# wtsi-svi/ReadServer

Hardware: AMD Instinct MI355X
Metric: 31-mer backward-search queries/sec on popBWT, counted as (query x shard) backward searches/s (higher is better)
Workload: dtype u64

## Files before the change

readserver_amd/csrc/search_lines.hip:

```cpp
#include <hip/hip_runtime.h>
#include <stdint.h>
#include <stdlib.h>
#include <string.h>

#include <type_traits>

#include "kernels.h"
#include "line_format.h"
#include "rank_device.h"
#include "wave_lines.h"

namespace rsb {


__device__ __forceinline__ ulonglong2 start_record(const shard_view &ix, const uint64_t *pq, uint32_t k) {
    ulonglong2 rec;
    const uint64_t last = pq[(k - 1u) >> 5];
    if (view_uses_ktab(ix, k)) {
        const uint32_t T = ix.ktab_depth;
        const uint32_t off = 2u * (k - T);
        const uint32_t w0 = off >> 6, sh = off & 63u;
        uint64_t bits = (w0 == ((k - 1u) >> 5) ? last : pq[w0]) >> sh;
        if (sh + 2u * T > 64u) bits |= last << (64u - sh);
        const uint64_t e = ktab_entry(ix.ktab, ix.ktab_fmt, T, ix.ktab_stride, bits & ((1ull << (2u * T)) - 1ull));
        const uint32_t width = (uint32_t)(e >> COUNT_BITS);
        if (width != KTAB_WIDE && (e & COUNT_MASK) + width <= ix.n) {
            rec.x = e & COUNT_MASK;
            rec.y = rec.x + width - 1ull;
            return rec;
        }
    }
    const uint32_t b = (uint32_t)((last >> (2u * ((k - 1u) & 31u))) & 3u) + 1u;
    rec.x = ix.C[b] | INIT_FALLBACK;
    rec.y = ix.C[b] + ix.total[b] - 1ull;
    return rec;
}

__global__ void __launch_bounds__(256)
search_init_kernel(const shard_view *__restrict__ shards, uint32_t nshards, const uint64_t *__restrict__ packed,
                   const uint8_t *__restrict__ valid, size_t Q, uint32_t k, uint32_t wpq,
                   ulonglong2 *__restrict__ init) {
    const size_t i = (size_t)blockIdx.x * blockDim.x + threadIdx.x;
    if (i >= Q * nshards) return;
    const size_t q = i / nshards, s = i - q * nshards;
    ulonglong2 rec;
    if (valid[q] == 0) {
        rec.x = INIT_INVALID;
        rec.y = 0;
    } else {
        rec = start_record(shards[s], packed + q * wpq, k);
    }
    init[s * Q + q] = rec;
}

__global__ void __launch_bounds__(256)
search_init_var_kernel(const shard_view *__restrict__ shards, uint32_t nshards, const uint64_t *__restrict__ packed,
                       const uint8_t *__restrict__ valid, const uint32_t *__restrict__ len, size_t Q, uint32_t wpq,
                       ulonglong2 *__restrict__ init) {
    const size_t i = (size_t)blockIdx.x * blockDim.x + threadIdx.x;
    if (i >= Q * nshards) return;
    const size_t q = i / nshards, s = i - q * nshards;
    const uint32_t L = len[q];
    ulonglong2 rec;
    if (valid[q] == 0 || L == 0u) {
        rec.x = INIT_INVALID;
        rec.y = 0;
    } else {
        const shard_view &ix = shards[s];
        const uint64_t *pq = packed + q * wpq;
        bool tabulated = false;
        if (view_uses_ktab(ix, L)) {
            const uint32_t T = ix.ktab_depth;
            const uint32_t off = 2u * (L - T);
            const uint32_t w0 = off >> 6, sh = off & 63u;
            uint64_t bits = pq[w0] >> sh;
            if (sh + 2u * T > 64u) bits |= pq[w0 + 1u] << (64u - sh);
            const uint64_t e = ktab_entry(ix.ktab, ix.ktab_fmt, T, ix.ktab_stride, bits & ((1ull << (2u * T)) - 1ull));
            const uint32_t width = (uint32_t)(e >> COUNT_BITS);
            if (width != KTAB_WIDE && (e & COUNT_MASK) + width <= ix.n) {
                rec.x = (e & COUNT_MASK) | ((uint64_t)(L - T) << COUNT_BITS) | INIT_EXPLICIT | INIT_VAR;
                rec.y = (e & COUNT_MASK) + width - 1ull;
                tabulated = true;
            }
        }
        if (!tabulated) {
            const uint32_t b = (uint32_t)((pq[(L - 1u) >> 5] >> (2u * ((L - 1u) & 31u))) & 3u) + 1u;
            rec.x = ix.C[b] | ((uint64_t)(L - 1u) << COUNT_BITS) | INIT_EXPLICIT | INIT_VAR | INIT_NOCHECK;
            rec.y = ix.C[b] + ix.total[b] - 1ull;
        }
    }
    init[s * Q + q] = rec;
}

__global__ void __launch_bounds__(256)
search_init_tiled_kernel(const shard_view *__restrict__ shards, uint32_t nshards, const uint64_t *__restrict__ packed,
                         const uint8_t *__restrict__ valid, size_t Q, uint32_t k, uint32_t wpq, uint32_t V,
                         ulonglong2 *__restrict__ init) {
    __shared__ ulonglong2 tile[256];
    const size_t q0 = (size_t)blockIdx.x * V;
    const uint32_t t = threadIdx.x;
    {
        const uint32_t v = t / nshards, s = t - v * nshards;
        if (v < V && q0 + v < Q) {
            const size_t q = q0 + v;
            ulonglong2 rec;
            if (valid[q] == 0) {
                rec.x = INIT_INVALID;
                rec.y = 0;
            } else {
                rec = start_record(shards[s], packed + q * wpq, k);
            }
            tile[v * nshards + s] = rec;
        }
    }
    __syncthreads();
    {
        const uint32_t s = t / V, v = t - s * V;
        if (s < nshards && q0 + v < Q) init[(size_t)s * Q + q0 + v] = tile[v * nshards + s];
    }
}

constexpr uint32_t INIT_U = 4;
__global__ void __launch_bounds__(256)
search_init_tiled4_kernel(const shard_view *__restrict__ shards, uint32_t nshards, const uint64_t *__restrict__ packed,
                          const uint8_t *__restrict__ valid, size_t Q, uint32_t k, uint32_t V, ulonglong2 *__restrict__ init) {
    __shared__ ulonglong2 tile[INIT_U][256];
    const size_t q0 = (size_t)blockIdx.x * V * INIT_U;
    const uint32_t t = threadIdx.x;
    {
        const uint32_t v = t / nshards, s = t - v * nshards;
        if (v < V) {
            const shard_view &ix = shards[s];
            const bool tab = view_uses_ktab(ix, k);
            const uint32_t T = ix.ktab_depth, off = tab ? 2u * (k - T) : 0u;
            const uint64_t *ktab = ix.ktab;
            const uint32_t fmt = ix.ktab_fmt, stride = ix.ktab_stride;
            const uint64_t n = ix.n;
            uint8_t ok[INIT_U];
            uint64_t word[INIT_U], e[INIT_U];
#pragma unroll
            for (uint32_t u = 0; u < INIT_U; ++u) {
                const size_t q = q0 + (size_t)u * V + v;
                const bool in = q < Q;
                ok[u] = in ? valid[q] : (uint8_t)2;
                word[u] = in ? packed[q] : 0ull;
            }
#pragma unroll
            for (uint32_t u = 0; u < INIT_U; ++u)
                e[u] = (tab && ok[u] == 1) ? ktab_entry(ktab, fmt, T, stride, (word[u] >> off) & ((1ull << (2u * T)) - 1ull)) : ~0ull;
#pragma unroll
            for (uint32_t u = 0; u < INIT_U; ++u) {
                if (ok[u] == 2) continue;
                ulonglong2 rec;
                const uint32_t width = (uint32_t)(e[u] >> COUNT_BITS);
                if (ok[u] == 0) {
                    rec.x = INIT_INVALID;
                    rec.y = 0;
                } else if (tab && width != KTAB_WIDE && (e[u] & COUNT_MASK) + width <= n) {
                    rec.x = e[u] & COUNT_MASK;
                    rec.y = rec.x + width - 1ull;
                } else {
                    const uint32_t b = (uint32_t)((word[u] >> (2u * ((k - 1u) & 31u))) & 3u) + 1u;
                    rec.x = ix.C[b] | INIT_FALLBACK;
                    rec.y = ix.C[b] + ix.total[b] - 1ull;
                }
                tile[u][v * nshards + s] = rec;
            }
        }
    }
    __syncthreads();
    {
        const uint32_t s = t / V, v = t - s * V;
        if (s < nshards) {
#pragma unroll
            for (uint32_t u = 0; u < INIT_U; ++u) {
                const size_t q = q0 + (size_t)u * V + v;
                if (q < Q) init[(size_t)s * Q + q] = tile[u][v * nshards + s];
            }
        }
    }
}

__global__ void __launch_bounds__(256)
search_init_1mm_kernel(const shard_view *__restrict__ shards, uint32_t nshards, const uint64_t *__restrict__ vpacked,
                       const uint8_t *__restrict__ vvalid, size_t mv, uint32_t k, uint32_t wpq, uint32_t V,
                       const ulonglong2 *__restrict__ trace, uint32_t trace_n,
                       ulonglong2 *__restrict__ init) {
    const size_t t_ = (size_t)blockIdx.x * blockDim.x + threadIdx.x;
    if (t_ >= mv * nshards) return;
    const size_t i = t_ / nshards, s = t_ - i * nshards;
    ulonglong2 rec;
    if (vvalid[i] == 0) {
        rec.x = INIT_INVALID;
        rec.y = 0;
    } else {
        const size_t q = i / V;
        const uint32_t v = (uint32_t)(i - q * V);
        const uint32_t pos = v ? (v - 1u) / 3u : ~0u;
        if (pos < trace_n) {
            const ulonglong2 t = trace[(s * (mv / V) + q) * trace_n + pos];
            rec.x = (t.x & COUNT_MASK) | ((uint64_t)pos << COUNT_BITS) | INIT_EXPLICIT;
            rec.y = t.y;
        } else {
            rec = start_record(shards[s], vpacked + i * wpq, k);
        }
    }
    init[s * mv + i] = rec;
}

enum { WORK_STEPS = 0, WORK_OCC = 1, WORK_LINES = 2, WORK_KTAB = 3, WORK_PHASE0 = 4, WORK_PASSES = 10, WORK_HOPS = 11, WORK_SOLO = 12 };
enum { WORK_UNSTAGED = 15 };

template <bool COUNT_WORK, bool COUNTS_ONLY, bool LONGK, int ROLE>
__global__ void __launch_bounds__(64 * WG_WAVES, RSB_MIN_WGS_PER_CU)
search_lines_kernel(const shard_view *__restrict__ shards, uint32_t nshards, const uint64_t *__restrict__ packed,
                    const ulonglong2 *__restrict__ init, unsigned long long *__restrict__ next_query,
                    size_t Q, uint32_t k, uint32_t wpq,
                    uint64_t *__restrict__ out_lower, uint64_t *__restrict__ out_upper,
                    unsigned long long *__restrict__ work,
                    ulonglong2 *__restrict__ trace, uint32_t trace_n, uint32_t qchunk, uint32_t pairs) {
    __shared__ uint4 s_stage[WG_WAVES][64 * SLOT_U4];
    const uint32_t lane = threadIdx.x & 63u;
    const uint32_t wave = threadIdx.x >> 6;
    const uint32_t side = lane >> 5;
    uint4 *stage = s_stage[wave];
    const uint32_t stage_lds = __builtin_amdgcn_readfirstlane((uint32_t)(uintptr_t)(lds_void_ptr)stage);
    const uint32_t swz = lane & 7u;
    const lds_u32 *own_row = reinterpret_cast<const lds_u32 *>(stage + (lane & 7u) * 64u + (lane >> 3) * SLOT_U4);
#define MINE(d) (mine0 + (((((uint32_t)(d)) >> 2) ^ swz) << 2) + (((uint32_t)(d)) & 3u))

    unsigned long long w_steps = 0, w_occ = 0, w_lines = 0, w_hops = 0, w_ktab = 0;
    unsigned long long ph[6] = {0, 0, 0, 0, 0, 0}, stamp = 0, passes = 0;
#define STAMP(i)                                                        \
    if (COUNT_WORK) {                                                   \
        __builtin_amdgcn_sched_barrier(0);                              \
        const unsigned long long now_ = __builtin_amdgcn_s_memtime();   \
        asm volatile("s_waitcnt lgkmcnt(0)" ::: "memory");              \
        ph[i] += now_ - stamp;                                          \
        stamp = now_;                                                   \
        __builtin_amdgcn_sched_barrier(0);                              \
    }
    if (COUNT_WORK) stamp = __builtin_amdgcn_s_memtime();

    uint32_t sid = blockIdx.x % nshards;
    for (uint32_t visited = 0; visited < nshards; ++visited, sid = (sid + 1u == nshards) ? 0u : sid + 1u) {
        const shard_view *sv = shards + sid;
        const char *lines_bytes = reinterpret_cast<const char *>(sv->lines);
        const uint32_t S = sv->sp.S;
        const double inv = sv->sp.inv;
        const uint32_t nlines = (uint32_t)sv->nlines;
        const bool ktab = view_uses_ktab(*sv, k);
        const int j_table = ktab ? (int)(k - sv->ktab_depth) - 1 : (int)k - 2;
        const uint32_t w_table = j_table > 0 ? (uint32_t)j_table >> 5 : 0u;
        const ulonglong2 *init_s = init + (size_t)sid * Q;
        uint64_t *out_lo = out_lower + (size_t)sid * Q * (pairs ? 2u : 1u);
        uint64_t *out_up = (COUNTS_ONLY || pairs) ? nullptr : out_upper + (size_t)sid * Q;
        unsigned long long *pool = next_query + (size_t)sid * POOL_STRIDE;
        if (visited != 0u && __hip_atomic_load(pool, __ATOMIC_RELAXED, __HIP_MEMORY_SCOPE_AGENT) >= (unsigned long long)Q) continue;
        ulonglong2 *trace_s = trace ? trace + (size_t)sid * Q * trace_n : nullptr;
        unsigned long long *hit_map = pairs == 2u ? reinterpret_cast<unsigned long long *>(out_upper) + (size_t)sid * hit_map_words(Q) : nullptr;
        uint32_t ctab_lo, ctab_hi;
        {
            const uint64_t c1 = sv->C[1], c2 = sv->C[2], c3 = sv->C[3], c4 = sv->C[4];
// ... 252 lines not shown
                has_n = true;
            }
            if (alive && done) {
                if (trace && side == 0u) {
                    for (int jj = j < (int)trace_n ? j : (int)trace_n - 1; jj >= 0; --jj)
                        trace_s[q * trace_n + (uint32_t)jj] = make_ulonglong2(lo, hi);
                }
                if (side == 0u) {
                    if (COUNTS_ONLY) {
                        if (hi >= lo) out_lo[q] = hi - lo + 1ull;
                    } else if (pairs == 2u) {
                        if (lo <= hi) {
                            reinterpret_cast<ulonglong2 *>(out_lo)[q] = make_ulonglong2(lo, hi);
                            atomicOr(hit_map + (q >> 6), 1ull << (q & 63u));
                        }
                    } else if (pairs) {
#ifdef RSB_NT_RESULTS
                        __builtin_nontemporal_store(lo, &out_lo[2 * q]);
                        __builtin_nontemporal_store(hi, &out_lo[2 * q + 1]);
#else
                        reinterpret_cast<ulonglong2 *>(out_lo)[q] = make_ulonglong2(lo, hi);
#endif
                    } else {
                        out_lo[q] = lo;
                        out_up[q] = hi;
                    }
                }
                has_q = false;
            }
            STAMP(5)
            if (COUNT_WORK) ++passes;
        }
    }
    if (COUNT_WORK) {
        if (lane == 0u) {
            for (int i = 0; i < 6; ++i) atomicAdd(&work[WORK_PHASE0 + i], ph[i]);
            atomicAdd(&work[WORK_PASSES], passes);
        }
        if (w_steps) atomicAdd(&work[WORK_STEPS], w_steps);
        if (w_occ) atomicAdd(&work[WORK_OCC], w_occ);
        if (w_lines) atomicAdd(&work[WORK_LINES], w_lines);
        if (w_ktab) atomicAdd(&work[WORK_KTAB], w_ktab);
        if (w_hops) atomicAdd(&work[WORK_HOPS], w_hops);
    }
#undef MINE
#undef STAMP
}

}
#include "search_solo.h"
namespace rsb {

static int search_kernel_choice() {
    static const int choice = [] {
        const char *e = getenv("RSBWT_SEARCH_KERNEL");
        if (e && !strcmp(e, "pair")) return SEARCH_PAIR;
        if (e && !strcmp(e, "solo")) return SEARCH_SOLO;
        return SEARCH_AUTO;
    }();
    return choice;
}

static size_t wave_wgs_per_cu() {
    static const size_t v = (size_t)knob_int("RSBWT_WAVE_WGS_PER_CU", 1, INT_MAX, RSB_MIN_WGS_PER_CU);
    return v;
}

static size_t search_cap(int num_cus, size_t wgs_per_cu) {
    static const size_t spare = (size_t)knob_int("RSBWT_SEARCH_SPARE_WGS", 1, LLONG_MAX, 0);
    return resident_cap(num_cus, wgs_per_cu, spare);
}

template <class F>
static void with_flag(bool b, F &&f) {
    if (b) f(std::true_type{});
    else f(std::false_type{});
}
#define FLAG(x) decltype(x)::value

template <bool CW, bool CO>
static void launch_solo(int grid, hipStream_t stream, const shard_view *shards, uint32_t nshards, const uint64_t *pk,
                        const ulonglong2 *init, const uint8_t *valid, unsigned long long *ctr, size_t Q, uint32_t k, uint32_t wpq,
                        uint64_t *lo, uint64_t *up, unsigned long long *work, ulonglong2 *trace, uint32_t trace_n,
                        uint32_t pairs, bool fused) {
    const uint32_t qchunk = plan_draw(1024, 64, (size_t)grid * WG_WAVES, 4, Q * nshards);
    static const bool no_staged = knob_set("RSBWT_NO_STAGED_RESULTS");
    const bool staged = !CO && pairs != 2u && !no_staged;
    static const bool count_unstaged = knob_set("RSBWT_COUNT_UNSTAGED");
    const uint32_t pa = pairs | (staged ? SOLO_STAGED_RESULTS : 0u) | (CW && count_unstaged ? SOLO_COUNT_UNSTAGED : 0u);
    const size_t dyn = staged ? SOLO_RESULTS_LDS : 0u;
    if (fused)
        hipLaunchKernelGGL((search_solo_kernel<CW, CO, false, true>), dim3(grid), dim3(64 * WG_WAVES), dyn, stream, shards, nshards,
                           pk, init, valid, ctr, Q, k, wpq, lo, up, work, trace, trace_n, qchunk, pa);
    else if (wpq > 1)
        hipLaunchKernelGGL((search_solo_kernel<CW, CO, true>), dim3(grid), dim3(64 * WG_WAVES), dyn, stream, shards, nshards,
                           pk, init, valid, ctr, Q, k, wpq, lo, up, work, trace, trace_n, qchunk, pa);
    else
        hipLaunchKernelGGL((search_solo_kernel<CW, CO, false>), dim3(grid), dim3(64 * WG_WAVES), dyn, stream, shards, nshards,
                           pk, init, valid, ctr, Q, k, wpq, lo, up, work, trace, trace_n, qchunk, pa);
}

template <bool CW, bool CO>
static void launch_k(int grid, hipStream_t stream, const shard_view *shards, uint32_t nshards, const uint64_t *pk,
                     const ulonglong2 *init, unsigned long long *ctr, size_t Q, uint32_t k, uint32_t wpq,
                     uint64_t *lo, uint64_t *up, unsigned long long *work, ulonglong2 *trace, uint32_t trace_n,
                     uint32_t pairs) {
    const uint32_t qchunk = plan_draw(1024, 32, (size_t)grid * WG_WAVES, 4, Q * nshards);
    if (wpq > 1)
        hipLaunchKernelGGL((search_lines_kernel<CW, CO, true, 0>), dim3(grid), dim3(64 * WG_WAVES), 0, stream, shards, nshards,
                           pk, init, ctr, Q, k, wpq, lo, up, work, trace, trace_n, qchunk, pairs);
    else
        hipLaunchKernelGGL((search_lines_kernel<CW, CO, false, 0>), dim3(grid), dim3(64 * WG_WAVES), 0, stream, shards, nshards,
                           pk, init, ctr, Q, k, wpq, lo, up, work, trace, trace_n, qchunk, pairs);
}

static void launch_init(const shard_view *d_shards, uint32_t nshards, const uint64_t *pk, const uint8_t *vd, size_t Q, uint32_t k,
                        uint32_t wpq, ulonglong2 *init, hipStream_t stream) {
    static const bool untiled = knob_set("RSBWT_INIT_UNTILED");
    static const bool one_per_thread = knob_set("RSBWT_INIT_ONE_PER_THREAD");
    if (nshards >= 2u && nshards <= 256u && !untiled && wpq == 1u && !one_per_thread) {
        const uint32_t V = 256u / nshards;
        hipLaunchKernelGGL(search_init_tiled4_kernel, dim3((unsigned)((Q + (size_t)V * INIT_U - 1) / ((size_t)V * INIT_U))), dim3(256), 0, stream,
                           d_shards, nshards, pk, vd, Q, k, V, init);
    } else if (nshards >= 2u && nshards <= 256u && !untiled) {
        const uint32_t V = 256u / nshards;
        hipLaunchKernelGGL(search_init_tiled_kernel, dim3((unsigned)((Q + V - 1) / V)), dim3(256), 0, stream, d_shards, nshards, pk, vd, Q,
                           k, wpq, V, init);
    } else {
        const size_t nrec = Q * nshards;
        hipLaunchKernelGGL(search_init_kernel, dim3((unsigned)((nrec + 255) / 256)), dim3(256), 0, stream, d_shards, nshards, pk, vd, Q, k,
                           wpq, init);
    }
}

hipError_t launch_search_init_var(const shard_view *d_shards, uint32_t nshards, const void *d_packed, const void *d_valid,
                                  const void *d_len, size_t Q, uint32_t wpq, void *d_init, hipStream_t stream) {
    if (Q == 0 || nshards == 0) return hipSuccess;
    const size_t nrec = Q * nshards;
    hipLaunchKernelGGL(search_init_var_kernel, dim3((unsigned)((nrec + 255) / 256)), dim3(256), 0, stream, d_shards, nshards,
                       (const uint64_t *)d_packed, (const uint8_t *)d_valid, (const uint32_t *)d_len, Q, wpq, (ulonglong2 *)d_init);
    return hipGetLastError();
}

hipError_t launch_search_init(const shard_view *d_shards, uint32_t nshards, const void *d_packed, const void *d_valid, size_t Q,
                              uint32_t k, void *d_init, hipStream_t stream) {
    if (Q == 0 || nshards == 0) return hipSuccess;
    const uint32_t wpq = (k + 31u) / 32u ? (k + 31u) / 32u : 1u;
    launch_init(d_shards, nshards, (const uint64_t *)d_packed, (const uint8_t *)d_valid, Q, k, wpq, (ulonglong2 *)d_init, stream);
    return hipGetLastError();
}

hipError_t launch_search(scratch_cache &scratch, const shard_view *d_shards, uint32_t nshards, const void *d_packed,
                         const void *d_valid, size_t Q, uint32_t k, void *d_lower, void *d_upper, bool counts_only,
                         unsigned long long *d_work, int num_cus, hipStream_t stream, hipEvent_t ev0, hipEvent_t ev1,
                         const search_extra *extra) {
    if (Q == 0 || nshards == 0) return hipSuccess;
    if (extra && extra->table_build && nshards != 1) return hipErrorInvalidValue;
    const bool hit_list = extra && extra->d_hit_bits && !counts_only;
    const uint32_t pairs = hit_list ? 2u : (extra && extra->pairs && !counts_only) ? 1u : 0u;
    ulonglong2 *trace = extra ? (ulonglong2 *)extra->d_trace_out : nullptr;
    const uint32_t trace_n = extra ? extra->trace_n : 0u;
    const uint32_t wpq = (k + 31u) / 32u ? (k + 31u) / 32u : 1u;
    const bool table_build = extra && extra->table_build, resumed = extra && extra->d_trace_in;
    const size_t nrec = Q * nshards;
    const size_t cap = search_cap(num_cus, wave_wgs_per_cu());
    const bool solo = plan_lone_lanes(search_kernel_choice(), table_build, nrec, cap, WG_WAVES, resumed, extra && extra->narrow);
    const int grid = (int)plan_grid(nrec, (solo ? 64u : 32u) * WG_WAVES, cap);
    const uint64_t *pk = (const uint64_t *)d_packed;
    const uint8_t *vd = (const uint8_t *)d_valid;
    uint64_t *lo = (uint64_t *)d_lower, *up = hit_list ? (uint64_t *)extra->d_hit_bits : (uint64_t *)d_upper;
    static const bool no_fused_start = knob_set("RSBWT_NO_FUSED_START");
    const bool fused = solo && nshards == 1 && extra && extra->narrow && !extra->d_init && !resumed && !trace && wpq == 1 && !no_fused_start;
    const bool prepared = (extra && extra->d_init) || fused;
    if (counts_only) {
        const hipError_t e = hipMemsetAsync(d_lower, 0, nrec * sizeof(uint64_t), stream);
        if (e != hipSuccess) return e;
    }
    pool_lease mem(scratch, stream, prepared ? 0 : nrec * sizeof(ulonglong2), 1, nshards);
    if (mem.error() != hipSuccess) return mem.error();
    ulonglong2 *init = fused ? nullptr : prepared ? (ulonglong2 *)extra->d_init : (ulonglong2 *)mem.front();
    unsigned long long *ctr = mem.pool(0, nshards);
    const unsigned ig = (unsigned)((nrec + 255) / 256);
    if (prepared) {
    } else if (resumed)
        hipLaunchKernelGGL(search_init_1mm_kernel, dim3(ig), dim3(256), 0, stream, d_shards, nshards, pk, vd, Q, k, wpq,
                           extra->variants, (const ulonglong2 *)extra->d_trace_in, trace_n, init);
    else
        launch_init(d_shards, nshards, pk, vd, Q, k, wpq, init, stream);
    if (ev0) (void)hipEventRecord(ev0, stream);
    if (table_build && !d_work && !counts_only && wpq == 1) {
        const uint32_t qchunk = plan_draw(1024, 32, (size_t)grid * WG_WAVES, 4, nrec);
        hipLaunchKernelGGL((search_lines_kernel<false, false, false, 1>), dim3(grid), dim3(64 * WG_WAVES), 0, stream, d_shards,
                           nshards, pk, init, ctr, Q, k, wpq, lo, up, d_work, trace, trace_n, qchunk, 0u);
    } else {
        with_flag(d_work != nullptr, [&](auto cw) {
            with_flag(counts_only, [&](auto co) {
                if (solo)
                    launch_solo<FLAG(cw), FLAG(co)>(grid, stream, d_shards, nshards, pk, init, vd, ctr, Q, k, wpq, lo, up, d_work, trace,
                                                    trace_n, pairs, fused);
                else
                    launch_k<FLAG(cw), FLAG(co)>(grid, stream, d_shards, nshards, pk, init, ctr, Q, k, wpq, lo, up, d_work, trace, trace_n,
                                                 pairs);
            });
        });
    }
    const hipError_t e = hipGetLastError();
    if (ev1) (void)hipEventRecord(ev1, stream);
    return e;
}

hipError_t launch_search_worklist(scratch_cache &scratch, const shard_view *d_shards, uint32_t nshards, const void *d_packed,
                                  const void *d_valid, size_t m, uint32_t tn, const void *d_worklists, const void *d_counts, size_t wl_cap,
                                  uint32_t k, void *d_sparse, void *d_hit_bits, unsigned long long *d_work, int num_cus,
                                  hipStream_t stream, hipEvent_t ev0, hipEvent_t ev1, const void *d_pre) {
    if (nshards == 0 || m == 0) return hipSuccess;
    if (k > 32u || tn == 0 || tn >= k) return hipErrorInvalidValue;
    const size_t implicit = m * 3u * (size_t)(k - tn), mv = m * (3u * (size_t)k + 1u);
    const size_t g = plan_grid((implicit + wl_cap) * nshards, 64u * WG_WAVES, search_cap(num_cus, wave_wgs_per_cu()));
    pool_lease mem(scratch, stream, 0, 1, nshards);
    if (mem.error() != hipSuccess) return mem.error();
    if (ev0) (void)hipEventRecord(ev0, stream);
    if (d_pre) {
        const hipError_t e = launch_wl_table_entries(d_shards, nshards, d_packed, m, k, tn, const_cast<void *>(d_pre), stream);
        if (e != hipSuccess) return e;
    }
    const uint32_t qchunk = plan_draw(1024, 64, g * WG_WAVES, 4, implicit * nshards);
    with_flag(d_work != nullptr, [&](auto cw) {
        hipLaunchKernelGGL((search_solo_kernel<FLAG(cw), false, false, false, true>), dim3((unsigned)g), dim3(64 * WG_WAVES), 0, stream, d_shards,
                           nshards, (const uint64_t *)d_packed, (const ulonglong2 *)d_worklists, (const uint8_t *)d_valid, mem.pool(0, nshards), mv,
                           k, 1u, (uint64_t *)d_sparse, (uint64_t *)d_hit_bits, d_work, (ulonglong2 *)const_cast<void *>(d_pre), tn, qchunk, 2u,
                           (const unsigned long long *)d_counts, wl_cap, implicit);
    });
    const hipError_t e = hipGetLastError();
    if (ev1) (void)hipEventRecord(ev1, stream);
    return e;
}

hipError_t launch_search_walk(scratch_cache &scratch, const shard_view *d_shards, uint32_t nshards, const void *d_packed,
                              const void *d_valid, size_t m, uint32_t tn, void *d_worklists, void *d_counts, size_t wl_cap, uint32_t k,
                              void *d_sparse, void *d_hit_bits, unsigned long long *d_work, int num_cus, hipStream_t stream,
                              hipEvent_t ev0, hipEvent_t ev1) {
    if (nshards == 0 || m == 0) return hipSuccess;
    if (k > 32u || tn == 0 || tn >= k) return hipErrorInvalidValue;
    static const size_t wgs_per_cu = (size_t)knob_int("RSBWT_WALK1MM_WGS_PER_CU", 1, RSB_WALK1MM_WGS_PER_CU, RSB_WALK1MM_WGS_PER_CU);
    const size_t g = plan_grid(m * nshards, 64u * WG_WAVES, search_cap(num_cus, wgs_per_cu));
    pool_lease mem(scratch, stream, 0, 1, nshards);
    if (mem.error() != hipSuccess) return mem.error();
    if (ev0) (void)hipEventRecord(ev0, stream);
    const uint32_t qchunk = plan_draw(1024, 64, g * WG_WAVES, 4, m * nshards);
    with_flag(d_work != nullptr, [&](auto cw) {
        hipLaunchKernelGGL((search_solo_kernel<FLAG(cw), false, false, true, false, true>), dim3((unsigned)g), dim3(64 * WG_WAVES), 0, stream,
                           d_shards, nshards, (const uint64_t *)d_packed, (const ulonglong2 *)d_worklists, (const uint8_t *)d_valid,
                           mem.pool(0, nshards), m, k, 1u, (uint64_t *)d_sparse, (uint64_t *)d_hit_bits, d_work, (ulonglong2 *)nullptr, tn, qchunk,
                           2u, (const unsigned long long *)d_counts, wl_cap, (size_t)0);
    });
    const hipError_t e = hipGetLastError();
    if (ev1) (void)hipEventRecord(ev1, stream);
    return e;
}
#undef FLAG

uint32_t trace_entries(const shard_view &ix, uint32_t k) {
    const bool ktab = ix.ktab != nullptr && ix.ktab_depth >= 2 && k >= ix.ktab_depth;
    if (!ktab || k <= ix.ktab_depth || k - ix.ktab_depth > 0xFFFFu) return 0;
    return k - ix.ktab_depth;
}

}
```

readserver_amd/csrc/search_solo.h:

```cpp
#ifndef RSBWT_SEARCH_SOLO_H
#define RSBWT_SEARCH_SOLO_H

namespace rsb {

constexpr uint64_t WL_DEAD = 1ull << 63;
constexpr uint32_t SOLO_STAGED_RESULTS = 4u;
constexpr uint32_t SOLO_COUNT_UNSTAGED = 8u;
constexpr uint32_t RES_WAVE_LDS = 2048u;
constexpr uint32_t SOLO_RESULTS_LDS = WG_WAVES * RES_WAVE_LDS;
constexpr uint32_t RES_SLOT_BYTES = 8u;
constexpr uint32_t RES_STATE_BYTES = 8u;
constexpr uint32_t RES_BUFS = RES_WAVE_LDS / (8u * RES_SLOT_BYTES + RES_STATE_BYTES);
static_assert(RES_BUFS * (8u * RES_SLOT_BYTES + RES_STATE_BYTES) <= RES_WAVE_LDS, "a wave's buffers and their state fit its 2 KB");
static_assert(RES_WAVE_LDS == 2048u && RES_BUFS == 28u, "2 KB per wave: with the line slots a CU's 160 KB at four workgroups");
static_assert(RES_BUFS >= 9u && RES_BUFS <= 32u, "the free buffers are a 32-bit mask; at most 9 groups begin among a pass's 64 draws");
constexpr uint32_t RES_NONE = 0xFFu;
constexpr uint32_t RES_WIDTH_BITS = 24u;
constexpr uint32_t RES_ESCAPED = (1u << RES_WIDTH_BITS) - 1u;

__device__ __forceinline__ void solo_lds_handoff() {
    __builtin_amdgcn_fence(__ATOMIC_RELEASE, "wavefront", "local");
    __builtin_amdgcn_wave_barrier();
    __builtin_amdgcn_fence(__ATOMIC_ACQUIRE, "wavefront", "local");
}

#ifndef RSB_WALK1MM_WGS_PER_CU
#define RSB_WALK1MM_WGS_PER_CU 3
#endif
template <bool COUNT_WORK, bool COUNTS_ONLY, bool LONGK, bool FUSED = false, bool WL = false, bool WALK = false>
__global__ void __launch_bounds__(64 * WG_WAVES, WALK ? RSB_WALK1MM_WGS_PER_CU : RSB_MIN_WGS_PER_CU)
search_solo_kernel(const shard_view *__restrict__ shards, uint32_t nshards, const uint64_t *__restrict__ packed,
                   const ulonglong2 *__restrict__ init, const uint8_t *__restrict__ valid,
                   unsigned long long *__restrict__ next_query,
                   size_t Q, uint32_t k, uint32_t wpq,
                   uint64_t *__restrict__ out_lower, uint64_t *__restrict__ out_upper,
                   unsigned long long *__restrict__ work,
                   ulonglong2 *__restrict__ trace, uint32_t trace_n, uint32_t qchunk, uint32_t pairs_arg,
                   const unsigned long long *__restrict__ wl_counts = nullptr, size_t wl_cap = 0, size_t wl_implicit = 0) {
    __shared__ uint4 s_stage[WG_WAVES][64 * SLOT_U4];
    extern __shared__ uint4 s_results[];
    const uint32_t lane = threadIdx.x & 63u;
    const uint32_t wave = threadIdx.x >> 6;
    uint4 *stage = s_stage[wave];
    const uint32_t stage_lds = __builtin_amdgcn_readfirstlane((uint32_t)(uintptr_t)(lds_void_ptr)stage);
    const uint32_t swz = lane & 7u;
    const uint32_t pairs = pairs_arg & 3u;
    constexpr bool CAN_STAGE = !COUNTS_ONLY && !WL && !WALK;
    const bool stage_out = CAN_STAGE && (pairs_arg & SOLO_STAGED_RESULTS) != 0u && pairs != 2u && Q < (1ull << 34);
    uint2 *results = reinterpret_cast<uint2 *>(s_results + wave * (RES_WAVE_LDS / 16u));
    uint32_t *res_state = reinterpret_cast<uint32_t *>(results + RES_BUFS * 8u);
    const bool count_unstaged = COUNT_WORK && (pairs_arg & SOLO_COUNT_UNSTAGED) != 0u;
    const lds_u32 *mine0 = reinterpret_cast<const lds_u32 *>(stage + (lane & 7u) * 64u + (lane >> 3) * SLOT_U4);
#define SOLO_MINE(d) (mine0 + (((((uint32_t)(d)) >> 2) ^ swz) << 2) + (((uint32_t)(d)) & 3u))

    unsigned long long w_steps = 0, w_occ = 0, w_lines = 0, w_hops = 0, w_ktab = 0, passes = 0;
    unsigned long long w_surv = 0, w_unstepped = 0;
    unsigned long long w_unstaged = 0;

    uint32_t sid = blockIdx.x % nshards;
    for (uint32_t visited = 0; visited < nshards; ++visited, sid = (sid + 1u == nshards) ? 0u : sid + 1u) {
        const shard_view *sv = shards + sid;
        const char *lines_bytes = reinterpret_cast<const char *>(sv->lines);
        const uint32_t S = sv->sp.S;
        const double inv = sv->sp.inv;
        const uint32_t nlines = (uint32_t)sv->nlines;
        const bool ktab = view_uses_ktab(*sv, k);
        const int j_table = ktab ? (int)(k - sv->ktab_depth) - 1 : (int)k - 2;
        const uint32_t w_table = j_table > 0 ? (uint32_t)j_table >> 5 : 0u;
        const ulonglong2 *init_s = WL ? init + (size_t)sid * wl_cap * 2u : init + (size_t)sid * Q;
        const size_t Qs = WALK ? Q : WL ? wl_implicit + (size_t)(wl_counts[(size_t)sid * WL_COUNT_STRIDE] < wl_cap ? wl_counts[(size_t)sid * WL_COUNT_STRIDE] : wl_cap) : Q;
        const uint32_t wl_tn = trace_n, wl_per = WL ? 3u * (k - trace_n) : 1u;
        const size_t walk_V = 3u * (size_t)k + 1u, walk_mv = Q * walk_V;
        ulonglong2 *walk_wl = WALK ? const_cast<ulonglong2 *>(init) + (size_t)sid * wl_cap * 2u : nullptr;
        unsigned long long *walk_count = WALK ? const_cast<unsigned long long *>(wl_counts) + (size_t)sid * WL_COUNT_STRIDE : nullptr;
        uint64_t *out_lo = WALK ? out_lower + (size_t)sid * walk_mv * 2u : out_lower + (size_t)sid * Q * (pairs ? 2u : 1u);
        uint64_t *out_up = (COUNTS_ONLY || pairs) ? nullptr : out_upper + (size_t)sid * Q;
        unsigned long long *pool = next_query + (size_t)sid * POOL_STRIDE;
        if (visited != 0u && __hip_atomic_load(pool, __ATOMIC_RELAXED, __HIP_MEMORY_SCOPE_AGENT) >= (unsigned long long)Qs) continue;
        ulonglong2 *trace_s = (trace && !WL) ? trace + (size_t)sid * Q * trace_n : nullptr;
        const uint64_t *wl_pre = (WL && trace) ? reinterpret_cast<const uint64_t *>(trace) + (size_t)sid * wl_implicit : nullptr;
        unsigned long long *hit_map = pairs == 2u ? reinterpret_cast<unsigned long long *>(out_upper) + (size_t)sid * hit_map_words(WALK ? walk_mv : Q) : nullptr;
        uint32_t ctab_lo, ctab_hi;
        {
            const uint64_t c1 = sv->C[1], c2 = sv->C[2], c3 = sv->C[3], c4 = sv->C[4];
            const uint32_t l3 = lane & 3u;
            const uint64_t cv = l3 == 0u ? c1 : l3 == 1u ? c2 : l3 == 2u ? c3 : c4;
            ctab_lo = (uint32_t)cv;
            ctab_hi = (uint32_t)(cv >> 32);
        }

        const uint64_t *__restrict__ ktab_p = sv->ktab;
        const uint32_t ktab_T = sv->ktab_depth, ktab_stride = sv->ktab_stride, ktab_fmt = sv->ktab_fmt;
        const uint64_t ix_n = sv->n;
        const uint64_t sc1 = sv->C[1], sc2 = sv->C[2], sc3 = sv->C[3], sc4 = sv->C[4];
        const uint64_t st1 = sv->total[1], st2 = sv->total[2], st3 = sv->total[3], st4 = sv->total[4];

        const uint32_t QCHUNK = qchunk;
        if (CAN_STAGE && stage_out && lane < RES_BUFS) {
            res_state[2u * lane + 1u] = 0u;
        }
        uint32_t res_buf = RES_NONE | (RES_NONE << 8);
        uint32_t open_g = ~0u, open_b = RES_NONE;
        uint64_t pool_next = 0, pool_end = 0;
        bool drained = false;
        size_t q = 0;
        bool has_q = false;
        size_t nq = 0;
        bool has_n = false;
        ulonglong2 nrec = {0, 0};
        uint64_t nword = 0;
        uint32_t nstage = 0;
        bool nimp = false;
        int j = 0;
        uint64_t word = 0, lo = 0, hi = 0;
        uint32_t sub = 0;
        uint64_t occL = 0, cacc = 0;
        uint32_t cont = 0, cblk = 0, cdw = 0, co = 0, tries = 0, w = 0;
        constexpr uint32_t SAME_WINDOW = 1u << 31;
        uint64_t altL0 = 0, altL1 = 0, altL2 = 0, altU0 = 0, altU1 = 0, altU2 = 0;
        bool alt_ok = true;

        for (;;) {
            bool done = false;
            bool last_in = false;
            if (FUSED && !has_q && has_n && nstage == 2u) {
                const uint64_t e = nrec.x;
                const uint32_t width = (uint32_t)(e >> COUNT_BITS);
                if (nrec.y == 0ull) {
                    nrec.x = INIT_INVALID;
                } else if (width != KTAB_WIDE && (e & COUNT_MASK) + width <= ix_n) {
                    nrec.x = e & COUNT_MASK;
                    nrec.y = nrec.x + width - 1ull;
                } else {
                    const uint32_t bl = (uint32_t)((nword >> (2u * ((k - 1u) & 31u))) & 3u);
                    const uint64_t cb = bl == 0u ? sc1 : bl == 1u ? sc2 : bl == 2u ? sc3 : sc4;
                    const uint64_t tb = bl == 0u ? st1 : bl == 1u ? st2 : bl == 2u ? st3 : st4;
                    nrec.x = cb | INIT_FALLBACK;
                    nrec.y = cb + tb - 1ull;
                }
            }
            if (WL && !has_q && has_n && nstage == 2u) {
                has_q = true;
                has_n = false;
                sub = 0;
                cont = 0;
                word = nword;
                if (nimp) {
                    const uint32_t r_ = (uint32_t)(nrec.y >> 8) & 0xFFu, q_ = (uint32_t)(nrec.y >> 32);
                    const uint32_t pr = (r_ * 171u) >> 9;
                    q = (size_t)q_ * (3u * k + 1u) + 1u + 3u * (wl_tn + pr) + (r_ - 3u * pr);
                    const uint64_t e = nrec.x;
                    const uint32_t width = (uint32_t)(e >> COUNT_BITS);
                    bool tabulated = false;
                    if (width != KTAB_WIDE && (e & COUNT_MASK) + width <= ix_n) {
                        lo = e & COUNT_MASK;
                        hi = lo + width - 1ull;
                        j = (int)wl_tn - 1;
                        tabulated = true;
                    } else {
                        const uint32_t bl = (uint32_t)((nword >> (2u * ((k - 1u) & 31u))) & 3u);
                        const uint64_t cb = bl == 0u ? sc1 : bl == 1u ? sc2 : bl == 2u ? sc3 : sc4;
                        const uint64_t tb = bl == 0u ? st1 : bl == 1u ? st2 : bl == 2u ? st3 : st4;
                        lo = cb;
                        hi = cb + tb - 1ull;
                        j = (int)k - 2;
                    }
                    done = (nrec.y & 0xFFull) == 0ull || (tabulated && lo > hi) || j < 0;
                } else {
                    q = nq;
                    lo = nrec.x & COUNT_MASK;
                    hi = nrec.y;
                    j = (int)((nrec.x >> COUNT_BITS) & 0xFFFFull);
                    done = (nrec.x & WL_DEAD) != 0ull || lo > hi;
                }
                if (done) { lo = 1; hi = 0; }
            }
            if (!WL && !has_q && has_n && (!FUSED || nstage == 2u)) {
                has_q = true;
                has_n = false;
                q = nq;
                if (CAN_STAGE) res_buf >>= 8;
                sub = 0;
                cont = 0;
                if (nrec.x & INIT_INVALID) {
                    lo = 1;
                    hi = 0;
                    j = -1;
                    done = true;
                } else if (nrec.x & INIT_EXPLICIT) {
                    lo = nrec.x & COUNT_MASK;
                    hi = nrec.y;
                    j = (int)((nrec.x >> COUNT_BITS) & 0xFFFFull) - ((nrec.x & INIT_VAR) ? 1 : 0);
                    word = nword;
                    done = j < 0 || ((nrec.x & INIT_NOCHECK) == 0ull && lo > hi);
                    if (LONGK) {
                        if (!done && ((uint32_t)j >> 5) != w_table) word = packed[q * wpq + ((uint32_t)j >> 5)];
                    }
                } else {
                    const bool fallback = !ktab || (nrec.x & INIT_FALLBACK) != 0ull;
                    lo = nrec.x & COUNT_MASK;
                    hi = nrec.y;
                    j = fallback ? (int)k - 2 : j_table;
                    word = nword;
                    if (COUNT_WORK && !fallback) w_ktab += 1;
                    done = (j < 0) || (!fallback && lo > hi);
                    if (LONGK) {
                        if (!done && ((uint32_t)j >> 5) != w_table) word = packed[q * wpq + ((uint32_t)j >> 5)];
                    }
                }
            }
            if (pool_next >= pool_end && !drained) {
                unsigned long long c = 0;
                if (lane == 0u) c = atomicAdd(pool, (unsigned long long)QCHUNK);
                c = ((unsigned long long)__builtin_amdgcn_readfirstlane((uint32_t)(c >> 32)) << 32) |
                    __builtin_amdgcn_readfirstlane((uint32_t)c);
                pool_next = c;
                pool_end = c + QCHUNK < Qs ? c + QCHUNK : Qs;
                if (c >= Qs) { drained = true; pool_next = pool_end = 0; }
            }
            bool got_n = false;
            {
                const uint64_t want_mask = __builtin_amdgcn_ballot_w64(!has_n);
                const uint32_t before = (uint32_t)__builtin_popcountll(want_mask & ((1ull << lane) - 1ull));
                const uint64_t mine = pool_next + before;
                if (!has_n && mine < pool_end) {
                    nq = (size_t)mine;
                    got_n = true;
                }
                const uint64_t taken = pool_next + (uint32_t)__builtin_popcountll(want_mask);
                const uint64_t r0 = pool_next;
                pool_next = taken < pool_end ? taken : pool_end;
                if (CAN_STAGE && stage_out && pool_next > r0) {
                    const uint32_t gq = (uint32_t)(nq >> 3);
                    uint32_t nb = gq == open_g ? open_b : RES_NONE;
                    const uint64_t first = (r0 + 7ull) & ~7ull;
                    if (first < pool_next) {
                        const uint32_t ga = (uint32_t)(first >> 3), gb = (uint32_t)((pool_next - 1ull) >> 3) + 1u;
                        uint32_t free_bufs = (uint32_t)__builtin_amdgcn_ballot_w64(lane < RES_BUFS && res_state[2u * lane + 1u] == 0u);
                        for (uint32_t g = ga; g < gb; ++g) {
                            const uint32_t bsel = free_bufs != 0u ? (uint32_t)__builtin_ctz(free_bufs) : RES_NONE;
                            free_bufs &= free_bufs - 1u;
                            if (gq == g) nb = bsel;
                            if (lane == bsel) {
                                const uint64_t q0 = (uint64_t)g << 3;
                                res_state[2u * lane + 1u] = (uint32_t)((q0 + 8ull < pool_end ? q0 + 8ull : pool_end) - q0);
                            }
                            open_b = bsel;
                        }
                        open_g = gb - 1u;
                    }
                    if (got_n) res_buf = (res_buf & 0xFFu) | (nb << 8);
                    solo_lds_handoff();
                }
            }
            if (__builtin_amdgcn_ballot_w64(has_q || got_n || ((FUSED || WL) && has_n)) == 0ull) {
                if (drained) break;
                continue;
            }
            ulonglong2 rec = {0, 0};
            uint64_t first_word = 0;
            const bool stage_b = (FUSED || WL) && has_n && nstage == 1u;
            uint64_t entry = 0;
            uint64_t wl_index = 0, vword = 0;
            bool imp = false;
            if (WL) {
                if (got_n) {
                    imp = nq < wl_implicit;
                    if (imp) {
                        const uint32_t i32 = (uint32_t)nq, q_ = i32 / wl_per, r_ = i32 - q_ * wl_per;
                        first_word = packed[q_];
                        rec.y = (uint64_t)valid[q_] | ((uint64_t)r_ << 8) | ((uint64_t)q_ << 32);
                    } else {
                        const size_t slot = nq - wl_implicit;
                        rec = init_s[2u * slot];
                        const ulonglong2 r2 = init_s[2u * slot + 1u];
                        wl_index = r2.x;
                        first_word = r2.y;
                    }
                }
                if (stage_b) {
                    const uint32_t r_ = (uint32_t)(nrec.y >> 8) & 0xFFu;
                    const uint32_t pr = (r_ * 171u) >> 9, d_ = r_ - 3u * pr, p_ = wl_tn + pr;
                    const uint32_t orig = (uint32_t)((nword >> (2u * p_)) & 3u);
                    const uint32_t alt = d_ < orig ? d_ : d_ + 1u;
                    vword = nword ^ ((uint64_t)(orig ^ alt) << (2u * p_));
                    const uint64_t code = (vword >> (2u * wl_tn)) & ((1ull << (2u * ktab_T)) - 1ull);
                    entry = wl_pre ? wl_pre[nq] : ktab_entry(ktab_p, ktab_fmt, ktab_T, ktab_stride, code);
                }
            } else if (FUSED) {
                if (got_n) {
                    rec.y = valid[nq];
                    first_word = packed[nq];
                }
                if (stage_b) {
                    const uint64_t code = (nword >> (2u * (k - ktab_T))) & ((1ull << (2u * ktab_T)) - 1ull);
                    entry = ktab_entry(ktab_p, ktab_fmt, ktab_T, ktab_stride, code);
                }
            } else if (got_n) {
                rec = init_s[nq];
                first_word = packed[nq * wpq + w_table];
            }
            const bool alive = has_q;
            const bool stepping = alive && !done;
            const bool fresh = stepping && cont == 0u;

            uint32_t b = 1, line = 0, o = 0;
            if (stepping) {
                if (LONGK) {
                    if (fresh && sub == 0u && (j & 31) == 31) word = packed[q * wpq + ((uint32_t)j >> 5)];
                }
                b = (uint32_t)((word >> (2u * ((uint32_t)j & 31u))) & 3u) + 1u;
            }
            bool no_fetch = false;
            if (fresh) {
                if (sub == 0u) {
                    if (WALK) {
                        alt_ok = true;
                        altL0 = altL1 = altL2 = altU0 = altU1 = altU2 = 0;
                    }
                    if (trace_s && (uint32_t)j < trace_n) trace_s[q * trace_n + (uint32_t)j] = make_ulonglong2(lo, hi);
                    if (lo == 0ull) {
                        occL = 0;
                        sub = 1u;
                    }
                }
                const uint64_t p = sub ? hi : lo - 1ull;
                if (p == ~0ull) {
                    no_fetch = true;
                } else {
                    uint32_t pin;
                    w = fast_window(p, S, inv, pin);
                    line = w + (w >> GROUP_SHIFT);
                    o = pin + 1u;
                    if (line >= nlines) line = 0;
                    if (COUNT_WORK) w_occ += 1;
                    if (sub == 0u) tries = hi - p <= (uint64_t)(S - o) ? SAME_WINDOW : 0u;
                }
            }
            const bool looking = stepping && !no_fetch;
            const uint64_t pb = ((uint64_t)(uint32_t)__builtin_amdgcn_ds_bpermute((int)((b - 1u) << 2), (int)ctab_hi) << 32) |
                                (uint32_t)__builtin_amdgcn_ds_bpermute((int)((b - 1u) << 2), (int)ctab_lo);

            const uint32_t want = looking ? (cont ? cblk : line) : ~0u;
            if (COUNT_WORK && want != ~0u) {
                if (cont) w_hops += 1;
                else w_lines += 1;
            }
            glds_fetch(lines_bytes, want, lane, stage_lds);
            glds_wait();

            bool do_scan = false, own_line = false;
            uint64_t base = 0;
            uint32_t dw = HDR_DWORDS, rem = 0;
            uint32_t s1 = 0, s2 = 0, s3 = 0, span = 0, hb = 0;
            const sym_tab stab = make_sym_tab(b);
            const uint32_t cont_in = cont;
            uint32_t more = 0;
            if (looking) {
                if (cont != KIND_CHUNK) {
                    if (cont == 0u) co = o;
                    const uint32_t oe = co;
                    const uint2 cw = *reinterpret_cast<const lds_u2 *>(SOLO_MINE(2u * (b - 1u)));
                    const uint4 h0 = *reinterpret_cast<const lds_u4 *>(SOLO_MINE(0));
                    const uint64_t cnt = ((uint64_t)(cw.y & 0xFFu) << 32) | cw.x;
                    const uint32_t m0 = h0.y >> 8, m1 = h0.w >> 8;
                    s1 = m0 & 0x3FFu;
                    s2 = (m0 >> 10) & 0x7FFu;
                    s3 = s2 + (m1 & 0x3FFu);
                    span = s3 + ((m1 >> 10) & 0x3FFu);
                    const uint32_t kind = (m1 >> 20) & 3u;
                    cacc = cnt;
                    if (kind == KIND_FAR) {
                        cblk = *SOLO_MINE(LINE_DWORDS - 1u);
                        if (cblk >= nlines) cblk = 0;
                        more = KIND_FAR;
                    } else if (kind == KIND_CHUNK && cont == 0u) {
                        const uint32_t m2 = *SOLO_MINE(5) >> 8, m3 = *SOLO_MINE(7) >> 8;
                        cdw = 2u * (((m2 >> 22) & 3u) | (((m3 >> 22) & 3u) << 2));
                        cblk = (w >> GROUP_SHIFT) * (GROUP + 1u) + GROUP;
// ... 278 lines not shown
```

Measured before the change: 4.426 billion.

## Use compact 8-byte block records for search init with wave-cooperative prefetch

```diff
diff --git a/readserver_amd/csrc/block_records.h b/readserver_amd/csrc/block_records.h
--- /dev/null
+++ b/readserver_amd/csrc/block_records.h
@@ -0,0 +1,37 @@
+#ifndef RSBWT_BLOCK_RECORDS_H
+#define RSBWT_BLOCK_RECORDS_H
+
+#include <stddef.h>
+#include <stdint.h>
+
+#include "line_format.h"
+
+namespace rsb {
+
+constexpr uint64_t BREC_WIDE = (uint64_t)KTAB_WIDE << COUNT_BITS;
+constexpr uint64_t BREC_INVALID = BREC_WIDE | COUNT_MASK;
+constexpr uint32_t BREC_BLOCK = 64;
+constexpr size_t BREC_ALIGN = 16;
+
+RSB_HD size_t brec_qpad(size_t Q) { return (Q + (BREC_ALIGN - 1)) & ~(BREC_ALIGN - 1); }
+RSB_HD size_t brec_bytes(size_t Q, size_t nshards) { return brec_qpad(Q) * nshards * sizeof(uint64_t); }
+
+RSB_HD uint64_t brec_encode(bool valid, bool tabulated, uint64_t entry, uint64_t n) {
+    if (!valid) return BREC_INVALID;
+    const uint32_t width = (uint32_t)(entry >> COUNT_BITS);
+    if (!tabulated || width == KTAB_WIDE || (entry & COUNT_MASK) + width > n) return BREC_WIDE;
+    return entry;
+}
+
+enum brec_kind { BREC_KIND_INTERVAL = 0, BREC_KIND_WIDE = 1, BREC_KIND_INVALID = 2 };
+RSB_HD brec_kind brec_decode(uint64_t rec, uint64_t &lower, uint64_t &upper) {
+    if (rec == BREC_INVALID) return BREC_KIND_INVALID;
+    const uint32_t width = (uint32_t)(rec >> COUNT_BITS);
+    if (width == KTAB_WIDE) return BREC_KIND_WIDE;
+    lower = rec & COUNT_MASK;
+    upper = lower + width - 1ull;
+    return BREC_KIND_INTERVAL;
+}
+
+}
+#endif
diff --git a/readserver_amd/csrc/search_lines.hip b/readserver_amd/csrc/search_lines.hip
--- a/readserver_amd/csrc/search_lines.hip
+++ b/readserver_amd/csrc/search_lines.hip
@@ -5,6 +5,7 @@
 
 #include <type_traits>
 
+#include "block_records.h"
 #include "kernels.h"
 #include "line_format.h"
 #include "rank_device.h"
@@ -121,10 +122,12 @@
 }
 
 constexpr uint32_t INIT_U = 4;
-__global__ void __launch_bounds__(256)
-search_init_tiled4_kernel(const shard_view *__restrict__ shards, uint32_t nshards, const uint64_t *__restrict__ packed,
-                          const uint8_t *__restrict__ valid, size_t Q, uint32_t k, uint32_t V, ulonglong2 *__restrict__ init) {
-    __shared__ ulonglong2 tile[INIT_U][256];
+template <class REC>
+__device__ __forceinline__ void search_init_tiled4(const shard_view *__restrict__ shards, uint32_t nshards, const uint64_t *__restrict__ packed,
+                                                   const uint8_t *__restrict__ valid, size_t Q, size_t Qrow, uint32_t k, uint32_t V,
+                                                   REC *__restrict__ init) {
+    constexpr bool COMPACT = std::is_same<REC, uint64_t>::value;
+    __shared__ REC tile[INIT_U][256];
     const size_t q0 = (size_t)blockIdx.x * V * INIT_U;
     const uint32_t t = threadIdx.x;
     {
@@ -151,6 +154,10 @@
 #pragma unroll
             for (uint32_t u = 0; u < INIT_U; ++u) {
                 if (ok[u] == 2) continue;
+                if constexpr (COMPACT) {
+                    tile[u][v * nshards + s] = brec_encode(ok[u] == 1, tab, e[u], n);
+                    continue;
+                }
                 ulonglong2 rec;
                 const uint32_t width = (uint32_t)(e[u] >> COUNT_BITS);
                 if (ok[u] == 0) {
@@ -164,7 +171,7 @@
                     rec.x = ix.C[b] | INIT_FALLBACK;
                     rec.y = ix.C[b] + ix.total[b] - 1ull;
                 }
-                tile[u][v * nshards + s] = rec;
+                if constexpr (!COMPACT) tile[u][v * nshards + s] = rec;
             }
         }
     }
@@ -175,10 +182,36 @@
 #pragma unroll
             for (uint32_t u = 0; u < INIT_U; ++u) {
                 const size_t q = q0 + (size_t)u * V + v;
-                if (q < Q) init[(size_t)s * Q + q] = tile[u][v * nshards + s];
-            }
-        }
-    }
+                if (q < Q) init[(size_t)s * Qrow + q] = tile[u][v * nshards + s];
+            }
+        }
+    }
+}
+__global__ void __launch_bounds__(256)
+search_init_tiled4_kernel(const shard_view *__restrict__ shards, uint32_t nshards, const uint64_t *__restrict__ packed,
+                          const uint8_t *__restrict__ valid, size_t Q, uint32_t k, uint32_t V, ulonglong2 *__restrict__ init) {
+    search_init_tiled4<ulonglong2>(shards, nshards, packed, valid, Q, Q, k, V, init);
+}
+__global__ void __launch_bounds__(256)
+search_init_block_tiled4_kernel(const shard_view *__restrict__ shards, uint32_t nshards, const uint64_t *__restrict__ packed,
+                                const uint8_t *__restrict__ valid, size_t Q, uint32_t k, uint32_t V, uint64_t *__restrict__ init) {
+    search_init_tiled4<uint64_t>(shards, nshards, packed, valid, Q, brec_qpad(Q), k, V, init);
+}
+
+__global__ void __launch_bounds__(256)
+search_init_block_kernel(const shard_view *__restrict__ shards, uint32_t nshards, const uint64_t *__restrict__ packed,
+                         const uint8_t *__restrict__ valid, size_t Q, uint32_t k, uint64_t *__restrict__ init) {
+    const size_t i = (size_t)blockIdx.x * blockDim.x + threadIdx.x;
+    if (i >= Q * nshards) return;
+    const size_t q = i / nshards, s = i - q * nshards;
+    const shard_view &ix = shards[s];
+    const bool ok = valid[q] != 0, tab = view_uses_ktab(ix, k);
+    uint64_t e = 0;
+    if (ok && tab) {
+        const uint32_t T = ix.ktab_depth;
+        e = ktab_entry(ix.ktab, ix.ktab_fmt, T, ix.ktab_stride, (packed[q] >> (2u * (k - T))) & ((1ull << (2u * T)) - 1ull));
+    }
+    init[s * brec_qpad(Q) + q] = brec_encode(ok, tab, e, ix.n);
 }
 
 __global__ void __launch_bounds__(256)
@@ -597,7 +630,7 @@
 static void launch_solo(int grid, hipStream_t stream, const shard_view *shards, uint32_t nshards, const uint64_t *pk,
                         const ulonglong2 *init, const uint8_t *valid, unsigned long long *ctr, size_t Q, uint32_t k, uint32_t wpq,
                         uint64_t *lo, uint64_t *up, unsigned long long *work, ulonglong2 *trace, uint32_t trace_n,
-                        uint32_t pairs, bool fused) {
+                        uint32_t pairs, bool fused, bool block_records) {
     const uint32_t qchunk = plan_draw(1024, 64, (size_t)grid * WG_WAVES, 4, Q * nshards);
     static const bool no_staged = knob_set("RSBWT_NO_STAGED_RESULTS");
     const bool staged = !CO && pairs != 2u && !no_staged;
@@ -607,6 +640,9 @@
     if (fused)
         hipLaunchKernelGGL((search_solo_kernel<CW, CO, false, true>), dim3(grid), dim3(64 * WG_WAVES), dyn, stream, shards, nshards,
                            pk, init, valid, ctr, Q, k, wpq, lo, up, work, trace, trace_n, qchunk, pa);
+    else if (block_records)
+        hipLaunchKernelGGL((search_solo_kernel<CW, CO, false, false, false, false, true>), dim3(grid), dim3(64 * WG_WAVES), dyn, stream, shards,
+                           nshards, pk, init, valid, ctr, Q, k, wpq, lo, up, work, trace, trace_n, qchunk, pa);
     else if (wpq > 1)
         hipLaunchKernelGGL((search_solo_kernel<CW, CO, true>), dim3(grid), dim3(64 * WG_WAVES), dyn, stream, shards, nshards,
                            pk, init, valid, ctr, Q, k, wpq, lo, up, work, trace, trace_n, qchunk, pa);
@@ -630,10 +666,19 @@
 }
 
 static void launch_init(const shard_view *d_shards, uint32_t nshards, const uint64_t *pk, const uint8_t *vd, size_t Q, uint32_t k,
-                        uint32_t wpq, ulonglong2 *init, hipStream_t stream) {
+                        uint32_t wpq, ulonglong2 *init, hipStream_t stream, bool block_records = false) {
     static const bool untiled = knob_set("RSBWT_INIT_UNTILED");
     static const bool one_per_thread = knob_set("RSBWT_INIT_ONE_PER_THREAD");
-    if (nshards >= 2u && nshards <= 256u && !untiled && wpq == 1u && !one_per_thread) {
+    if (block_records) {
+        if (nshards >= 2u && nshards <= 256u && !untiled && !one_per_thread) {
+            const uint32_t V = 256u / nshards;
+            hipLaunchKernelGGL(search_init_block_tiled4_kernel, dim3((unsigned)((Q + (size_t)V * INIT_U - 1) / ((size_t)V * INIT_U))), dim3(256), 0,
+                               stream, d_shards, nshards, pk, vd, Q, k, V, (uint64_t *)init);
+        } else {
+            hipLaunchKernelGGL(search_init_block_kernel, dim3((unsigned)((Q * nshards + 255) / 256)), dim3(256), 0, stream, d_shards, nshards, pk,
+                               vd, Q, k, (uint64_t *)init);
+        }
+    } else if (nshards >= 2u && nshards <= 256u && !untiled && wpq == 1u && !one_per_thread) {
         const uint32_t V = 256u / nshards;
         hipLaunchKernelGGL(search_init_tiled4_kernel, dim3((unsigned)((Q + (size_t)V * INIT_U - 1) / ((size_t)V * INIT_U))), dim3(256), 0, stream,
                            d_shards, nshards, pk, vd, Q, k, V, init);
@@ -687,11 +732,13 @@
     static const bool no_fused_start = knob_set("RSBWT_NO_FUSED_START");
     const bool fused = solo && nshards == 1 && extra && extra->narrow && !extra->d_init && !resumed && !trace && wpq == 1 && !no_fused_start;
     const bool prepared = (extra && extra->d_init) || fused;
+    static const bool no_block_records = knob_set("RSBWT_NO_BLOCK_RECORDS");
+    const bool block_records = solo && wpq == 1 && !trace && !resumed && !prepared && !no_block_records;
     if (counts_only) {
         const hipError_t e = hipMemsetAsync(d_lower, 0, nrec * sizeof(uint64_t), stream);
         if (e != hipSuccess) return e;
     }
-    pool_lease mem(scratch, stream, prepared ? 0 : nrec * sizeof(ulonglong2), 1, nshards);
+    pool_lease mem(scratch, stream, prepared ? 0 : block_records ? brec_bytes(Q, nshards) : nrec * sizeof(ulonglong2), 1, nshards);
     if (mem.error() != hipSuccess) return mem.error();
     ulonglong2 *init = fused ? nullptr : prepared ? (ulonglong2 *)extra->d_init : (ulonglong2 *)mem.front();
     unsigned long long *ctr = mem.pool(0, nshards);
@@ -701,7 +748,7 @@
         hipLaunchKernelGGL(search_init_1mm_kernel, dim3(ig), dim3(256), 0, stream, d_shards, nshards, pk, vd, Q, k, wpq,
                            extra->variants, (const ulonglong2 *)extra->d_trace_in, trace_n, init);
     else
-        launch_init(d_shards, nshards, pk, vd, Q, k, wpq, init, stream);
+        launch_init(d_shards, nshards, pk, vd, Q, k, wpq, init, stream, block_records);
     if (ev0) (void)hipEventRecord(ev0, stream);
     if (table_build && !d_work && !counts_only && wpq == 1) {
         const uint32_t qchunk = plan_draw(1024, 32, (size_t)grid * WG_WAVES, 4, nrec);
@@ -712,7 +759,7 @@
             with_flag(counts_only, [&](auto co) {
                 if (solo)
                     launch_solo<FLAG(cw), FLAG(co)>(grid, stream, d_shards, nshards, pk, init, vd, ctr, Q, k, wpq, lo, up, d_work, trace,
-                                                    trace_n, pairs, fused);
+                                                    trace_n, pairs, fused, block_records);
                 else
                     launch_k<FLAG(cw), FLAG(co)>(grid, stream, d_shards, nshards, pk, init, ctr, Q, k, wpq, lo, up, d_work, trace, trace_n,
                                                  pairs);
diff --git a/readserver_amd/csrc/search_solo.h b/readserver_amd/csrc/search_solo.h
--- a/readserver_amd/csrc/search_solo.h
+++ b/readserver_amd/csrc/search_solo.h
@@ -27,7 +27,7 @@
 #ifndef RSB_WALK1MM_WGS_PER_CU
 #define RSB_WALK1MM_WGS_PER_CU 3
 #endif
-template <bool COUNT_WORK, bool COUNTS_ONLY, bool LONGK, bool FUSED = false, bool WL = false, bool WALK = false>
+template <bool COUNT_WORK, bool COUNTS_ONLY, bool LONGK, bool FUSED = false, bool WL = false, bool WALK = false, bool BLOCKREC = false>
 __global__ void __launch_bounds__(64 * WG_WAVES, WALK ? RSB_WALK1MM_WGS_PER_CU : RSB_MIN_WGS_PER_CU)
 search_solo_kernel(const shard_view *__restrict__ shards, uint32_t nshards, const uint64_t *__restrict__ packed,
                    const ulonglong2 *__restrict__ init, const uint8_t *__restrict__ valid,
@@ -68,6 +68,7 @@
         const int j_table = ktab ? (int)(k - sv->ktab_depth) - 1 : (int)k - 2;
         const uint32_t w_table = j_table > 0 ? (uint32_t)j_table >> 5 : 0u;
         const ulonglong2 *init_s = WL ? init + (size_t)sid * wl_cap * 2u : init + (size_t)sid * Q;
+        const uint64_t *brec_s = BLOCKREC ? reinterpret_cast<const uint64_t *>(init) + (size_t)sid * brec_qpad(Q) : nullptr;
         const size_t Qs = WALK ? Q : WL ? wl_implicit + (size_t)(wl_counts[(size_t)sid * WL_COUNT_STRIDE] < wl_cap ? wl_counts[(size_t)sid * WL_COUNT_STRIDE] : wl_cap) : Q;
         const uint32_t wl_tn = trace_n, wl_per = WL ? 3u * (k - trace_n) : 1u;
         const size_t walk_V = 3u * (size_t)k + 1u, walk_mv = Q * walk_V;
@@ -109,6 +110,7 @@
         bool has_n = false;
         ulonglong2 nrec = {0, 0};
         uint64_t nword = 0;
+        uint64_t brec = 0, bword = 0, bend = 0;
         uint32_t nstage = 0;
         bool nimp = false;
         int j = 0;
@@ -182,6 +184,20 @@
                 if (CAN_STAGE) res_buf >>= 8;
                 sub = 0;
                 cont = 0;
+                if (BLOCKREC) {
+                    uint64_t lower = 0, upper = 0;
+                    const brec_kind kind = brec_decode(nrec.x, lower, upper);
+                    if (kind == BREC_KIND_INVALID) {
+                        nrec = make_ulonglong2(INIT_INVALID, 0ull);
+                    } else if (kind == BREC_KIND_INTERVAL) {
+                        nrec = make_ulonglong2(lower, upper);
+                    } else {
+                        const uint32_t bl = (uint32_t)((nword >> (2u * ((k - 1u) & 31u))) & 3u);
+                        const uint64_t cb = bl == 0u ? sc1 : bl == 1u ? sc2 : bl == 2u ? sc3 : sc4;
+                        const uint64_t tb = bl == 0u ? st1 : bl == 1u ? st2 : bl == 2u ? st3 : st4;
+                        nrec = make_ulonglong2(cb | INIT_FALLBACK, cb + tb - 1ull);
+                    }
+                }
                 if (nrec.x & INIT_INVALID) {
                     lo = 1;
                     hi = 0;
@@ -217,19 +233,32 @@
                 pool_next = c;
                 pool_end = c + QCHUNK < Qs ? c + QCHUNK : Qs;
                 if (c >= Qs) { drained = true; pool_next = pool_end = 0; }
+                if (BLOCKREC && !drained) {
+                    const uint64_t i = c + lane;
+                    brec = i < Qs ? brec_s[i] : BREC_INVALID;
+                    bword = i < Qs ? packed[i] : 0ull;
+                    bend = c + BREC_BLOCK;
+                }
             }
             bool got_n = false;
+            uint32_t bsrc = 0;
+            bool bdrew = false;
             {
                 const uint64_t want_mask = __builtin_amdgcn_ballot_w64(!has_n);
                 const uint32_t before = (uint32_t)__builtin_popcountll(want_mask & ((1ull << lane) - 1ull));
                 const uint64_t mine = pool_next + before;
-                if (!has_n && mine < pool_end) {
+                const uint64_t draw_end = BLOCKREC && bend < pool_end ? bend : pool_end;
+                if (!has_n && mine < draw_end) {
                     nq = (size_t)mine;
                     got_n = true;
                 }
                 const uint64_t taken = pool_next + (uint32_t)__builtin_popcountll(want_mask);
                 const uint64_t r0 = pool_next;
-                pool_next = taken < pool_end ? taken : pool_end;
+                pool_next = taken < draw_end ? taken : draw_end;
+                if (BLOCKREC) {
+                    bsrc = ((uint32_t)mine - (uint32_t)bend) & (BREC_BLOCK - 1u);
+                    bdrew = pool_next > r0;
+                }
                 if (CAN_STAGE && stage_out && pool_next > r0) {
                     const uint32_t gq = (uint32_t)(nq >> 3);
                     uint32_t nb = gq == open_g ? open_b : RES_NONE;
@@ -295,6 +324,20 @@
                 if (stage_b) {
                     const uint64_t code = (nword >> (2u * (k - ktab_T))) & ((1ull << (2u * ktab_T)) - 1ull);
                     entry = ktab_entry(ktab_p, ktab_fmt, ktab_T, ktab_stride, code);
+                }
+            } else if (BLOCKREC) {
+                if (bdrew) {
+                    const int a = (int)(bsrc << 2);
+                    rec.x = ((uint64_t)(uint32_t)__builtin_amdgcn_ds_bpermute(a, (int)(uint32_t)(brec >> 32)) << 32) |
+                            (uint32_t)__builtin_amdgcn_ds_bpermute(a, (int)(uint32_t)brec);
+                    first_word = ((uint64_t)(uint32_t)__builtin_amdgcn_ds_bpermute(a, (int)(uint32_t)(bword >> 32)) << 32) |
+                                 (uint32_t)__builtin_amdgcn_ds_bpermute(a, (int)(uint32_t)bword);
+                    if (pool_next == bend && bend < pool_end) {
+                        const uint64_t i = bend + lane;
+                        brec = i < Qs ? brec_s[i] : BREC_INVALID;
+                        bword = i < Qs ? packed[i] : 0ull;
+                        bend += BREC_BLOCK;
+                    }
                 }
             } else if (got_n) {
                 rec = init_s[nq];
```

New measurement: 4.402 billion. About the same (-0.5%).
